# weidafeng/Efficient-SlowFast

Hardware: AMD Instinct MI355X
Metric: clips/sec (8x8 224^2 SlowFast-R50+CMDA, train step fwd+bwd+allreduce+SGD) (higher is better)
Workload: dtype f32

## Files before the change

efficient-slowfast_amd/csrc/conv_bx.hip:

```cpp
#include "bx.h"
#include <stdlib.h>

namespace {

constexpr int BXC_BM = 256;
constexpr int BXC_BK = 16;
constexpr int BXC_STAGES = 3;
constexpr int BXC_ROWB = BXC_BK * 2;
constexpr int BXC_A_STAGE = 3 * BXC_BM * BXC_ROWB;

struct BxArgs {
  sf_conv_desc d;
  const unsigned short* ap;
  const unsigned short* bp;
  float* ws;
  const float* scale;
  const float* bias;
  const float* res;
  float* out;
  int M, ntaps, cpk, nk, S, nk_per, nb_n, tiles;
  int tap_major;
  unsigned a_rows, a_bytes, b_bytes;
  unsigned a_plane, b_plane;
  unsigned wo_mul, wo_sh, ho_mul, ho_sh, to_mul, to_sh;
  const float* xf;
  unsigned xf_bytes;
  float* stats;
};

__device__ __forceinline__ unsigned mdiv(unsigned n, unsigned mul, unsigned sh) {
  return mul ? (__umulhi(n, mul) >> sh) : n;
}

typedef __attribute__((address_space(3))) void lds_void;

template <int BN, bool DIRECT, int VAR>
__global__ __launch_bounds__(512, 2) void conv_bx_kernel(const BxArgs p) {
  constexpr bool AF32 = (VAR & 32) != 0;
  constexpr int A_ST = AF32 ? BXC_BM * 64 : BXC_A_STAGE;
  constexpr int B_STAGE = 3 * BN * BXC_ROWB;
  constexpr int STAGE = A_ST + B_STAGE;
  constexpr int NT = BN / 64;
  extern __shared__ __attribute__((aligned(16))) char smem[];
  const sf_conv_desc& d = p.d;
  const int tid = threadIdx.x, lane = tid & 63;
  const int wave = __builtin_amdgcn_readfirstlane(tid >> 6);
  const int wm = wave & 3, wn = wave >> 2;
  const int bid = xcd_remap(blockIdx.x, p.tiles * p.S);
  const int split = bid / p.tiles, tile = bid - split * p.tiles;
  const int tile_m = tile / p.nb_n, tile_n = tile - tile_m * p.nb_n;
  const int m0 = tile_m * BXC_BM, n0 = tile_n * BN;
  const int ks0 = split * p.nk_per;
  const int ks1 = ks0 + p.nk_per < p.nk ? ks0 + p.nk_per : p.nk;
  const int nsteps = ks1 - ks0;

  const int lrow = lane >> 1;
  const unsigned lchunk = (unsigned)((lane & 1) ^ ((lrow >> 4) & 1)) * 16u;
  const int am = m0 + 32 * wave + lrow;
  const bool a_ok = am < p.M;
  int t0, h0, w0, nimg;
  {
    const unsigned mm = a_ok ? (unsigned)am : 0u;
    const unsigned q1 = mdiv(mm, p.wo_mul, p.wo_sh);
    const unsigned wo = mm - q1 * (unsigned)d.Wo;
    const unsigned q2 = mdiv(q1, p.ho_mul, p.ho_sh);
    const unsigned ho = q1 - q2 * (unsigned)d.Ho;
    const unsigned q3 = mdiv(q2, p.to_mul, p.to_sh);
    const unsigned to = q2 - q3 * (unsigned)d.To;
    nimg = (int)q3;
    t0 = d.transposed ? (int)to + d.pT : (int)to * d.sT - d.pT;
    h0 = d.transposed ? (int)ho + d.pH : (int)ho * d.sH - d.pH;
    w0 = d.transposed ? (int)wo + d.pW : (int)wo * d.sW - d.pW;
  }
  struct FRow { int t0, h0, w0, n; bool ok; unsigned chunk; };
  FRow fr0 = {0, 0, 0, 0, false, 0u}, fr1 = fr0;
  if constexpr (AF32) {
    auto frow = [&](int u) -> FRow {
      FRow f;
      const int r = 32 * wave + 16 * u + (lane >> 2);
      const int fm = m0 + r;
      f.ok = fm < p.M;
      f.chunk = (unsigned)((lane & 3) ^ ((r >> 2) & 3)) * 16u;
      const unsigned mm = f.ok ? (unsigned)fm : 0u;
      const unsigned q1 = mdiv(mm, p.wo_mul, p.wo_sh);
      const unsigned wo = mm - q1 * (unsigned)d.Wo;
      const unsigned q2 = mdiv(q1, p.ho_mul, p.ho_sh);
      const unsigned ho = q1 - q2 * (unsigned)d.Ho;
      const unsigned q3 = mdiv(q2, p.to_mul, p.to_sh);
      const unsigned to = q2 - q3 * (unsigned)d.To;
      f.n = (int)q3;
      f.t0 = d.transposed ? (int)to + d.pT : (int)to * d.sT - d.pT;
      f.h0 = d.transposed ? (int)ho + d.pH : (int)ho * d.sH - d.pH;
      f.w0 = d.transposed ? (int)wo + d.pW : (int)wo * d.sW - d.pW;
      return f;
    };
    fr0 = frow(0);
    fr1 = frow(1);
  }
  auto f_voff = [&](const FRow f, int kt, int kh, int kw) -> unsigned {
    const int ti = d.transposed ? f.t0 - kt * d.dT : f.t0 + kt * d.dT;
    const int hi = d.transposed ? f.h0 - kh * d.dH : f.h0 + kh * d.dH;
    const int wi = d.transposed ? f.w0 - kw * d.dW : f.w0 + kw * d.dW;
    const bool ok = f.ok && (unsigned)ti < (unsigned)d.Ti && (unsigned)hi < (unsigned)d.Hi && (unsigned)wi < (unsigned)d.Wi;
    if (!ok) return 0x80000000u;
    const unsigned r = (unsigned)(((f.n * d.Ti + ti) * d.Hi + hi) * d.Wi + wi);
    return (r * (unsigned)d.in_cs + (unsigned)d.in_coff) * 4u + f.chunk;
  };
  const unsigned row_bytes = (unsigned)d.Cin * 2u;
  auto a_voff = [&](int kt, int kh, int kw) -> unsigned {
    const int ti = d.transposed ? t0 - kt * d.dT : t0 + kt * d.dT;
    const int hi = d.transposed ? h0 - kh * d.dH : h0 + kh * d.dH;
    const int wi = d.transposed ? w0 - kw * d.dW : w0 + kw * d.dW;
    const bool ok = a_ok && (unsigned)ti < (unsigned)d.Ti && (unsigned)hi < (unsigned)d.Hi && (unsigned)wi < (unsigned)d.Wi;
    const unsigned r = ok ? (unsigned)(((nimg * d.Ti + ti) * d.Hi + hi) * d.Wi + wi) : p.a_rows;
    return r * row_bytes + lchunk;
  };
  const bool b_loader = BN == 256 || wave < BN / 32;
  const int bn = n0 + 32 * wave + lrow;
  const unsigned kbytes = (unsigned)p.nk * (unsigned)BXC_ROWB;
  const unsigned b_voff = (unsigned)((b_loader && bn < d.Cout) ? bn : d.Cout) * kbytes + lchunk;

  const __amdgpu_buffer_rsrc_t a_rs = __builtin_amdgcn_make_buffer_rsrc((void*)p.ap, 0, p.a_bytes, 0x00020000);
  const __amdgpu_buffer_rsrc_t b_rs = __builtin_amdgcn_make_buffer_rsrc((void*)p.bp, 0, p.b_bytes, 0x00020000);
  const __amdgpu_buffer_rsrc_t x_rs = __builtin_amdgcn_make_buffer_rsrc((void*)p.xf, 0, AF32 ? p.xf_bytes : 0u, 0x00020000);

  struct LS { int c, tap, kw, kh, kt; };
  LS ls;
  ls.c = __builtin_amdgcn_readfirstlane(p.tap_major ? ks0 % p.cpk : ks0 / p.ntaps);
  ls.tap = __builtin_amdgcn_readfirstlane(p.tap_major ? ks0 / p.cpk : ks0 - ls.c * p.ntaps);
  ls.kw = __builtin_amdgcn_readfirstlane(ls.tap % d.kW);
  ls.kh = __builtin_amdgcn_readfirstlane((ls.tap / d.kW) % d.kH);
  ls.kt = __builtin_amdgcn_readfirstlane(ls.tap / (d.kW * d.kH));
  const int tap_major = p.tap_major, cpk = p.cpk, kW = d.kW, kH = d.kH, kT = d.kT;
  auto next = [=](const LS o) -> LS {
    LS n;
    if (tap_major) {
      const int c1 = o.c + 1;
      const bool wc = c1 == cpk;
      n.c = wc ? 0 : c1;
      n.tap = o.tap + (wc ? 1 : 0);
      const int w1 = o.kw + (wc ? 1 : 0);
      const bool ww = w1 == kW;
      n.kw = ww ? 0 : w1;
      const int h1 = o.kh + (ww ? 1 : 0);
      const bool wh = h1 == kH;
      n.kh = wh ? 0 : h1;
      n.kt = o.kt + (wh ? 1 : 0);
      return n;
    }
    const int w1 = o.kw + 1;
    const bool ww = w1 == kW;
    n.kw = ww ? 0 : w1;
    const int h1 = o.kh + (ww ? 1 : 0);
    const bool wh = h1 == kH;
    n.kh = wh ? 0 : h1;
    const int t1 = o.kt + (wh ? 1 : 0);
    const bool wt = t1 == kT;
    n.kt = wt ? 0 : t1;
    n.tap = wt ? 0 : o.tap + 1;
    n.c = o.c + (wt ? 1 : 0);
    return n;
  };
  auto issue = [&](int stage) {
    const LS l = ls;
    unsigned cur_voff = 0, cur_aso, cur_f0 = 0, cur_f1 = 0;
    if constexpr (AF32) {
      cur_f0 = f_voff(fr0, l.kt, l.kh, l.kw);
      cur_f1 = f_voff(fr1, l.kt, l.kh, l.kw);
      cur_aso = (unsigned)l.c * 64u;
    } else {
      cur_voff = a_voff(l.kt, l.kh, l.kw);
      cur_aso = (unsigned)l.c * (unsigned)BXC_ROWB;
    }
    const unsigned cur_bso = (unsigned)(l.tap * p.cpk + l.c) * (unsigned)BXC_ROWB;
    if constexpr (AF32) {
      __builtin_amdgcn_raw_ptr_buffer_load_lds(x_rs, (lds_void*)(smem + stage * STAGE + wave * 2048), 16, cur_f0, cur_aso,
                                               0, 0);
      __builtin_amdgcn_raw_ptr_buffer_load_lds(x_rs, (lds_void*)(smem + stage * STAGE + wave * 2048 + 1024), 16, cur_f1,
                                               cur_aso, 0, 0);
    } else {
      char* const sa = smem + stage * STAGE + wave * 1024;
#pragma unroll
      for (int g = 0; g < 3; ++g)
        __builtin_amdgcn_raw_ptr_buffer_load_lds(a_rs, (lds_void*)(sa + g * (BXC_BM * BXC_ROWB)), 16, cur_voff,
                                                 cur_aso + (unsigned)g * p.a_plane, 0, 0);
    }
    if (b_loader) {
      char* const sb = smem + stage * STAGE + A_ST + wave * 1024;
#pragma unroll
      for (int g = 0; g < 3; ++g)
        __builtin_amdgcn_raw_ptr_buffer_load_lds(b_rs, (lds_void*)(sb + g * (BN * BXC_ROWB)), 16, b_voff,
                                                 cur_bso + (unsigned)g * p.b_plane, 0, 0);
    }
    ls = next(l);
  };

  const unsigned frag_lane = (unsigned)(lane & 31) * BXC_ROWB + (unsigned)(((lane >> 5) ^ ((lane >> 4) & 1)) * 16);
  const unsigned a_frag = (unsigned)(wm * 64) * BXC_ROWB + frag_lane;
  const unsigned b_frag = A_ST + (unsigned)(wn * (BN / 2)) * BXC_ROWB + frag_lane;
  unsigned f_frag[2][2] = {{0, 0}, {0, 0}};
  if constexpr (AF32) {
#pragma unroll
    for (int i = 0; i < 2; ++i) {
      const int r = wm * 64 + i * 32 + (lane & 31);
#pragma unroll
      for (int q = 0; q < 2; ++q) f_frag[i][q] = (unsigned)r * 64u + (unsigned)(((2 * (lane >> 5) + q) ^ ((r >> 2) & 3)) * 16);
    }
  }

  f32x16 acc[2][NT];
#pragma unroll
  for (int i = 0; i < 2; ++i)
#pragma unroll
    for (int j = 0; j < NT; ++j)
#pragma unroll
      for (int e = 0; e < 16; ++e) acc[i][j][e] = 0.f;

  if (nsteps > 0) issue(0);
  if (nsteps > 1) issue(1);
  for (int it = 0; it < nsteps; ++it) {
    if (it + 1 < nsteps) {
      if constexpr (AF32) {
        if (b_loader) asm volatile("s_waitcnt vmcnt(5)" ::: "memory");
        else asm volatile("s_waitcnt vmcnt(2)" ::: "memory");
      } else {
        if (b_loader) asm volatile("s_waitcnt vmcnt(6)" ::: "memory");
        else asm volatile("s_waitcnt vmcnt(3)" ::: "memory");
      }
    } else {
      asm volatile("s_waitcnt vmcnt(0)" ::: "memory");
    }
    __builtin_amdgcn_s_barrier();
    if (!(VAR & 16) && it + 2 < nsteps) issue((it + 2) % BXC_STAGES);
    const char* const st = smem + (it % BXC_STAGES) * STAGE;
    u32x4 af[2][3], bf[NT][3];
    if constexpr (AF32) {
#pragma unroll
      for (int i = 0; i < 2; ++i) {
        const f32x4 lo = *reinterpret_cast<const f32x4*>(st + f_frag[i][0]);
        const f32x4 hi = *reinterpret_cast<const f32x4*>(st + f_frag[i][1]);
        split_pair(lo[0], lo[1], af[i], 0);
        split_pair(lo[2], lo[3], af[i], 1);
        split_pair(hi[0], hi[1], af[i], 2);
        split_pair(hi[2], hi[3], af[i], 3);
      }
    }
#pragma unroll
    for (int pc = 0; pc < 3; ++pc) {
      if constexpr (!AF32) {
#pragma unroll
        for (int i = 0; i < 2; ++i)
          af[i][pc] = *reinterpret_cast<const u32x4*>(st + a_frag + pc * (BXC_BM * BXC_ROWB) + i * (32 * BXC_ROWB));
      }
#pragma unroll
      for (int j = 0; j < NT; ++j)
        bf[j][pc] = *reinterpret_cast<const u32x4*>(st + b_frag + pc * (BN * BXC_ROWB) + j * (32 * BXC_ROWB));
    }
    if (VAR & 8) {
      unsigned x = 0;
#pragma unroll
      for (int pc = 0; pc < 3; ++pc) {
#pragma unroll
        for (int i = 0; i < 2; ++i) x ^= af[i][pc][0] ^ af[i][pc][1] ^ af[i][pc][2] ^ af[i][pc][3];
#pragma unroll
        for (int j = 0; j < NT; ++j) x ^= bf[j][pc][0] ^ bf[j][pc][1] ^ bf[j][pc][2] ^ bf[j][pc][3];
      }
      acc[0][0][0] += __builtin_bit_cast(float, x & 0x007fffffu);
    } else {
#pragma unroll
      for (int i = 0; i < 2; ++i)
#pragma unroll
        for (int j = 0; j < NT; ++j) acc[i][j] = mfma_split(af[i], bf[j], acc[i][j]);
    }
  }

  const int col = lane & 31, rsub = 4 * (lane >> 5);
  if ((VAR & 4) && p.M > 0) {
    return;
  }
  if (DIRECT) {
#pragma unroll
    for (int j = 0; j < NT; ++j) {
      const int n = n0 + wn * (BN / 2) + j * 32 + col;
      const bool n_ok = n < d.Cout;
      const float sc = (p.scale && n_ok) ? p.scale[n] : 1.f;
      const float bi = (p.bias && n_ok) ? p.bias[n] : 0.f;
#pragma unroll
      for (int i = 0; i < 2; ++i) {
        float r[16];
#pragma unroll
        for (int e = 0; e < 16; ++e) {
          const int m = m0 + wm * 64 + i * 32 + (e & 3) + 8 * (e >> 2) + rsub;
          r[e] = (p.res && m < p.M && n_ok) ? p.res[(long)m * d.res_cs + d.res_coff + n] : 0.f;
        }
#pragma unroll
        for (int e = 0; e < 16; ++e) {
          const int m = m0 + wm * 64 + i * 32 + (e & 3) + 8 * (e >> 2) + rsub;
          if (m < p.M && n_ok) p.out[(long)m * d.out_cs + d.out_coff + n] = sf_act(acc[i][j][e] * sc + bi + r[e], d.act);
        }
      }
    }
    return;
  }
  float* const wsp = p.ws + (long)split * p.M * d.Cout;
#pragma unroll
  for (int i = 0; i < 2; ++i)
#pragma unroll
    for (int j = 0; j < NT; ++j) {
      const int n = n0 + wn * (BN / 2) + j * 32 + col;
#pragma unroll
      for (int e = 0; e < 16; ++e) {
        const int m = m0 + wm * 64 + i * 32 + (e & 3) + 8 * (e >> 2) + rsub;
        if (m < p.M && n < d.Cout) wsp[(long)m * d.Cout + n] = acc[i][j][e];
      }
    }
}

template <int BN, int ST>
__global__ __launch_bounds__(512, ST == 2 ? 4 : 2) void conv_pw_bx_kernel(const BxArgs p) {
  constexpr int A_STAGE = BXC_BM * 64;
  constexpr int B_STAGE = 3 * BN * BXC_ROWB;
  constexpr int STAGE = A_STAGE + B_STAGE;
  constexpr int NT = BN / 64;
  extern __shared__ __attribute__((aligned(16))) char smem[];
  const sf_conv_desc& d = p.d;
  const int tid = threadIdx.x, lane = tid & 63;
  const int wave = __builtin_amdgcn_readfirstlane(tid >> 6);
  const int wm = wave & 3, wn = wave >> 2;
  const int bid = xcd_remap(blockIdx.x, p.tiles);
  const int tile_m = bid / p.nb_n, tile_n = bid - tile_m * p.nb_n;
  const int m0 = tile_m * BXC_BM, n0 = tile_n * BN;
  const int nsteps = p.nk;

  const int lrow = lane >> 1;
  const unsigned lchunk = (unsigned)((lane & 1) ^ ((lrow >> 4) & 1)) * 16u;
  const bool b_loader = BN == 256 || wave < BN / 32;
  const int bn = n0 + 32 * wave + lrow;
  const unsigned kbytes = (unsigned)p.nk * (unsigned)BXC_ROWB;
  const unsigned b_voff = (unsigned)((b_loader && bn < d.Cout) ? bn : d.Cout) * kbytes + lchunk;
  const __amdgpu_buffer_rsrc_t b_rs = __builtin_amdgcn_make_buffer_rsrc((void*)p.bp, 0, p.b_bytes, 0x00020000);
  const __amdgpu_buffer_rsrc_t x_rs = __builtin_amdgcn_make_buffer_rsrc((void*)p.xf, 0, p.xf_bytes, 0x00020000);
  unsigned a_lvoff[2];
#pragma unroll
  for (int u = 0; u < 2; ++u) {
    const int r = 32 * wave + 16 * u + (lane >> 2);
    const int m = m0 + r;
    const unsigned chunk = (unsigned)((lane & 3) ^ ((r >> 2) & 3));
    a_lvoff[u] = m < p.M ? ((unsigned)m * (unsigned)d.in_cs + (unsigned)d.in_coff) * 4u + chunk * 16u : 0x80000000u;
  }
  auto issue = [&](int step) {
    char* const st = smem + (step % ST) * STAGE;
#pragma unroll
    for (int u = 0; u < 2; ++u)
      __builtin_amdgcn_raw_ptr_buffer_load_lds(x_rs, (lds_void*)(st + wave * 2048 + u * 1024), 16, a_lvoff[u],
                                               (unsigned)step * 64u, 0, 0);
    if (b_loader) {
      char* const sb = st + A_STAGE + wave * 1024;
#pragma unroll
      for (int g = 0; g < 3; ++g)
        __builtin_amdgcn_raw_ptr_buffer_load_lds(b_rs, (lds_void*)(sb + g * (BN * BXC_ROWB)), 16, b_voff,
                                                 (unsigned)step * (unsigned)BXC_ROWB + (unsigned)g * p.b_plane, 0, 0);
    }
  };
  unsigned a_frag[2][2];
#pragma unroll
  for (int i = 0; i < 2; ++i) {
    const int r = wm * 64 + i * 32 + (lane & 31);
#pragma unroll
    for (int q = 0; q < 2; ++q)
      a_frag[i][q] = (unsigned)r * 64u + (unsigned)(((2 * (lane >> 5) + q) ^ ((r >> 2) & 3)) * 16);
  }
  const unsigned frag_lane = (unsigned)(lane & 31) * BXC_ROWB + (unsigned)(((lane >> 5) ^ ((lane >> 4) & 1)) * 16);
  const unsigned b_frag = A_STAGE + (unsigned)(wn * (BN / 2)) * BXC_ROWB + frag_lane;

  f32x16 acc[2][NT];
#pragma unroll
  for (int i = 0; i < 2; ++i)
#pragma unroll
    for (int j = 0; j < NT; ++j)
#pragma unroll
      for (int e = 0; e < 16; ++e) acc[i][j][e] = 0.f;

  if (nsteps > 0) issue(0);
  if (ST == 3 && nsteps > 1) issue(1);
  for (int it = 0; it < nsteps; ++it) {
    if (ST == 3 && it + 1 < nsteps) {
      if (b_loader) asm volatile("s_waitcnt vmcnt(5)" ::: "memory");
      else asm volatile("s_waitcnt vmcnt(2)" ::: "memory");
    } else {
      asm volatile("s_waitcnt vmcnt(0)" ::: "memory");
    }
    __builtin_amdgcn_s_barrier();
    if (it + ST - 1 < nsteps) issue(it + ST - 1);
    const char* const st = smem + (it % ST) * STAGE;
    u32x4 af[2][3], bf[NT][3];
#pragma unroll
    for (int i = 0; i < 2; ++i) {
      const f32x4 lo = *reinterpret_cast<const f32x4*>(st + a_frag[i][0]);
      const f32x4 hi = *reinterpret_cast<const f32x4*>(st + a_frag[i][1]);
      split_pair(lo[0], lo[1], af[i], 0);
      split_pair(lo[2], lo[3], af[i], 1);
      split_pair(hi[0], hi[1], af[i], 2);
      split_pair(hi[2], hi[3], af[i], 3);
    }
#pragma unroll
    for (int pc = 0; pc < 3; ++pc)
#pragma unroll
      for (int j = 0; j < NT; ++j)
        bf[j][pc] = *reinterpret_cast<const u32x4*>(st + b_frag + pc * (BN * BXC_ROWB) + j * (32 * BXC_ROWB));
#pragma unroll
    for (int i = 0; i < 2; ++i)
#pragma unroll
      for (int j = 0; j < NT; ++j) acc[i][j] = mfma_split(af[i], bf[j], acc[i][j]);
  }

  const int col = lane & 31, rsub = 4 * (lane >> 5);
  const bool want_stats = p.stats != nullptr;
  float* const kred = reinterpret_cast<float*>(smem);
  if (want_stats) __syncthreads();
#pragma unroll
  for (int j = 0; j < NT; ++j) {
    const int cl = wn * (BN / 2) + j * 32 + col;
    const int n = n0 + cl;
    const bool n_ok = n < d.Cout;
    const float sc = (p.scale && n_ok) ? p.scale[n] : 1.f;
    const float bi = (p.bias && n_ok) ? p.bias[n] : 0.f;
#pragma unroll
    for (int i = 0; i < 2; ++i) {
      float r[16];
#pragma unroll
      for (int e = 0; e < 16; ++e) {
        const int m = m0 + wm * 64 + i * 32 + (e & 3) + 8 * (e >> 2) + rsub;
        r[e] = (p.res && m < p.M && n_ok) ? p.res[(long)m * d.res_cs + d.res_coff + n] : 0.f;
      }
#pragma unroll
      for (int e = 0; e < 16; ++e) {
        const int m = m0 + wm * 64 + i * 32 + (e & 3) + 8 * (e >> 2) + rsub;
        const float v = sf_act(acc[i][j][e] * sc + bi + r[e], d.act);
        acc[i][j][e] = v;
        if (m < p.M && n_ok) p.out[(long)m * d.out_cs + d.out_coff + n] = v;
      }
    }
    if (want_stats && wm == 0 && rsub == 0) kred[cl] = acc[0][j][0];
  }
  if (!want_stats) return;
  __syncthreads();
  float* const sred = kred + BN;
#pragma unroll
  for (int j = 0; j < NT; ++j) {
    const int cl = wn * (BN / 2) + j * 32 + col;
    const float k0 = kred[cl];
    float s1 = 0.f, s2 = 0.f;
#pragma unroll
    for (int i = 0; i < 2; ++i)
#pragma unroll
      for (int e = 0; e < 16; ++e) {
        const int m = m0 + wm * 64 + i * 32 + (e & 3) + 8 * (e >> 2) + rsub;
        if (m < p.M) {
          const float dv = acc[i][j][e] - k0;
          s1 += dv;
          s2 += dv * dv;
        }
      }
    s1 += __shfl_xor(s1, 32, 64);
    s2 += __shfl_xor(s2, 32, 64);
    if (rsub == 0) {
      sred[(wm * BN + cl) * 2] = s1;
      sred[(wm * BN + cl) * 2 + 1] = s2;
    }
  }
  __syncthreads();
  if (tid < BN) {
    const int n = n0 + tid;
    if (n < d.Cout) {
      float s1 = 0.f, s2 = 0.f;
#pragma unroll
      for (int w = 0; w < 4; ++w) {
        s1 += sred[(w * BN + tid) * 2];
        s2 += sred[(w * BN + tid) * 2 + 1];
      }
      const int left = p.M - m0;
      const float cnt = (float)(left < BXC_BM ? left : BXC_BM);
      float* const o = p.stats + ((long)tile_m * (d.Cout >> 2) + (n >> 2)) * 16 + (n & 3);
      o[0] = cnt;
      o[4] = kred[tid];
      o[8] = s1;
      o[12] = s2;
    }
  }
}

struct BxwArgs {
  sf_conv_desc d;
  const unsigned short* xp;
  const unsigned short* zp;
  float* part;
  int M, Kc, S, chunk, nb_col, tiles;
  unsigned x_rows, x_plane, x_bytes, z_plane, z_bytes;
  unsigned wo_mul, wo_sh, ho_mul, ho_sh, to_mul, to_sh, ci_mul, ci_sh;
};

__device__ __forceinline__ u32x2 lds_tr(const char* p) {
  return lds_read_tr(reinterpret_cast<const unsigned short*>(p));
}
__device__ __forceinline__ u32x2 lds_tr_raw(unsigned lds_byte_addr) {
  u32x2 r;
  asm volatile("ds_read_b64_tr_b16 %0, %1" : "=v"(r) : "v"(lds_byte_addr));
  return r;
}

template <int BCO>
__global__ __launch_bounds__(512, 2) void conv_bx_wgrad_kernel(const BxwArgs p) {
  constexpr int BCOL = 256;
  constexpr int NWC = BCO == 256 ? 2 : 4;
  constexpr int NT = BCOL / NWC / 32;
  constexpr int ROW_A = BCO * 2, ROW_B = BCOL * 2;
  constexpr int PL_A = 16 * ROW_A, PL_B = 16 * ROW_B;
  constexpr int A_STAGE = 3 * PL_A, STAGE = A_STAGE + 3 * PL_B;
  constexpr int NA = PL_A / 1024;
  constexpr int CPR_A = BCO / 8;
  extern __shared__ __attribute__((aligned(16))) char smem[];
  const sf_conv_desc& d = p.d;
  const int tid = threadIdx.x, lane = tid & 63;
  const int wave = __builtin_amdgcn_readfirstlane(tid >> 6);
  const int wr = wave / NWC, wc = wave - wr * NWC;
  const int bid = xcd_remap(blockIdx.x, p.tiles * p.S);
  const int split = bid / p.tiles, tile = bid - split * p.tiles;
  const int tile_co = tile / p.nb_col, tile_col = tile - tile_co * p.nb_col;
  const int co0 = tile_co * BCO, col0 = tile_col * BCOL;
  const int mb = split * p.chunk;
  const int me = mb + p.chunk < p.M ? mb + p.chunk : p.M;
  const int nsteps = me > mb ? (me - mb + 15) / 16 : 0;

  const int b_pos = 2 * wave + (lane >> 5);
  const int b_cs = (lane & 31) ^ ((b_pos & 3) << 2);
  const int b_col = col0 + b_cs * 8;
  const bool b_colok = b_col < p.Kc;
  const unsigned b_tap = b_colok ? mdiv((unsigned)b_col, p.ci_mul, p.ci_sh) : 0u;
  const unsigned b_ci = b_colok ? (unsigned)b_col - b_tap * (unsigned)d.Cin : 0u;
  const int b_kw = (int)(b_tap % (unsigned)d.kW), b_kh = (int)((b_tap / (unsigned)d.kW) % (unsigned)d.kH),
            b_kt = (int)(b_tap / (unsigned)(d.kW * d.kH));
  const int b_dt = b_kt * d.dT - d.pT, b_dh = b_kh * d.dH - d.pH, b_dw = b_kw * d.dW - d.pW;
  const unsigned x_rowb = (unsigned)d.Cin * 2u;
  auto b_voff = [&](int m) -> unsigned {
    unsigned r = p.x_rows;
    if (m < me && b_colok) {
      const unsigned q1 = mdiv((unsigned)m, p.wo_mul, p.wo_sh);
      const int wo = (int)((unsigned)m - q1 * (unsigned)d.Wo);
      const unsigned q2 = mdiv(q1, p.ho_mul, p.ho_sh);
      const int ho = (int)(q1 - q2 * (unsigned)d.Ho);
      const unsigned q3 = mdiv(q2, p.to_mul, p.to_sh);
      const int to = (int)(q2 - q3 * (unsigned)d.To);
      const int ti = to * d.sT + b_dt, hi = ho * d.sH + b_dh, wi = wo * d.sW + b_dw;
      if ((unsigned)ti < (unsigned)d.Ti && (unsigned)hi < (unsigned)d.Hi && (unsigned)wi < (unsigned)d.Wi)
        r = (unsigned)((((int)q3 * d.Ti + ti) * d.Hi + hi) * d.Wi + wi);
    }
    return r * x_rowb + b_ci * 2u;
  };
  const bool a_loader = wave < NA;
  const int a_pos = wave * (64 / CPR_A) + lane / CPR_A;
  const int a_cs = (lane % CPR_A) ^ ((a_pos & 3) << 2);
  const int a_co = co0 + a_cs * 8;
  const unsigned z_rowb = (unsigned)d.Cout * 2u;
  auto a_voff = [&](int m) -> unsigned {
    const unsigned r = (m < me && a_co < d.Cout) ? (unsigned)m : (unsigned)p.M;
    return r * z_rowb + (unsigned)(a_co < d.Cout ? a_co : 0) * 2u;
// ... 116 lines not shown
    } else {
      w[0] = w[1] = w[2] = (u32x4){0u, 0u, 0u, 0u};
    }
#pragma unroll
    for (int pc = 0; pc < 3; ++pc) *reinterpret_cast<u32x4*>(planes + pc * plane + r * C + c) = w[pc];
  }
}

struct BxSplitItem {
  const float* x;
  unsigned short* planes;
  long rows;
  int C, pad_;
};
__global__ __launch_bounds__(256) void bx_split_batched_kernel(const BxSplitItem* __restrict__ items,
                                                               const int* __restrict__ blk0, int n) {
  int lo = 0, hi = n;
  while (hi - lo > 1) {
    const int mid = (lo + hi) >> 1;
    if (blk0[mid] <= (int)blockIdx.x) lo = mid; else hi = mid;
  }
  const BxSplitItem it = items[lo];
  const int c8 = it.C >> 3;
  const long idx = (long)((int)blockIdx.x - blk0[lo]) * 256 + threadIdx.x;
  if (idx >= (it.rows + 1) * c8) return;
  const long plane = (it.rows + 1) * (long)it.C;
  const long r = idx / c8;
  const int c = (int)(idx - r * c8) * 8;
  u32x4 w[3];
  if (r < it.rows) {
    const f32x4 v0 = *reinterpret_cast<const f32x4*>(it.x + r * it.C + c);
    const f32x4 v1 = *reinterpret_cast<const f32x4*>(it.x + r * it.C + c + 4);
    split_pair(v0[0], v0[1], w, 0);
    split_pair(v0[2], v0[3], w, 1);
    split_pair(v1[0], v1[1], w, 2);
    split_pair(v1[2], v1[3], w, 3);
  } else {
    w[0] = w[1] = w[2] = (u32x4){0u, 0u, 0u, 0u};
  }
#pragma unroll
  for (int pc = 0; pc < 3; ++pc) *reinterpret_cast<u32x4*>(it.planes + pc * plane + r * it.C + c) = w[pc];
}

void magic(unsigned dv, unsigned* mul, unsigned* sh) {
  if (dv <= 1) { *mul = 0; *sh = 0; return; }
  unsigned l = 0;
  while ((1u << l) < dv) ++l;
  const unsigned long long num = 1ull << (31 + l);
  *mul = (unsigned)((num + dv - 1) / dv);
  *sh = l - 1;
}

int g_bx_enable = 1;
int g_bx_dbg = 0;

bool bx_enabled() {
  static const int env_on = [] {
    const char* e = getenv("SF_CONV_BX");
    return e ? atoi(e) : 1;
  }();
  return env_on && g_bx_enable;
}

struct BxPlan { int bn, S, nk, nk_per, nb_n, tiles, direct; long a_rows; };

bool bx_af32(const sf_conv_desc* d);

bool bx_plan(const sf_conv_desc* d, BxPlan* pl, bool gate = true) {
  if (!bx_enabled()) return false;
  const long M = (long)d->N * d->To * d->Ho * d->Wo;
  const int ntaps = d->kT * d->kH * d->kW;
  if ((d->Cin % 16) || d->cin_pad != d->Cin || (d->in_cs % 4) || (d->in_coff % 4)) return false;
  if (d->Cout < 128 || (d->Cout % 4) || d->out_cmul != 1) return false;
  const int nk = ntaps * (d->Cin / BXC_BK);
  if (nk < 32 || M < 2048 || M > 0x7fffffffL) return false;
  if (d->transposed && (d->sT != 1 || d->sH != 1 || d->sW != 1)) return false;
  const long a_rows = (long)d->N * d->Ti * d->Hi * d->Wi;
  if (3 * (a_rows + 1) * d->Cin * 2 > 0xfffffff0L) return false;
  if (3L * (d->Cout + 1) * nk * BXC_ROWB > 0xfffffff0L) return false;
  pl->bn = d->Cout >= 256 ? 256 : 128;
  pl->nb_n = sf_cdiv(d->Cout, pl->bn);
  pl->tiles = sf_cdiv(M, BXC_BM) * pl->nb_n;
  pl->nk = nk;
  pl->a_rows = a_rows;
  const bool scatter = d->os_T > 1 || d->os_H > 1 || d->os_W > 1;
  const double step_us = pl->bn == 256 ? 2.05 : 1.6;
  const double out_mb = (double)M * d->Cout * 4e-6;
  int best = 1;
  double best_t = 1e30;
  for (int S = 1; S <= 16 && nk / S >= 8; ++S) {
    const long wg = (long)pl->tiles * S;
    if (wg > 2048) break;
    const long rounds = sf_cdiv(wg, 256);
    double t = 6.0 + (double)rounds * sf_cdiv(nk, S) * step_us;
    if (S > 1 || scatter) t += 3.0 + out_mb * (2.0 * S + 1.0) / 4.0;
    else t += out_mb / 4.0;
    if (t < best_t - 1e-9) { best_t = t; best = S; }
  }
  static const int forced_s = [] { const char* e = getenv("SF_CONV_BX_S"); return e ? atoi(e) : 0; }();
  if (forced_s > 0 && nk / forced_s >= 1) best = forced_s;
  pl->S = best;
  pl->nk_per = sf_cdiv(nk, best);
  pl->direct = (best == 1 && !scatter) ? 1 : 0;
  if (gate && g_bx_enable < 2) {
    const double flop = 2.0 * M * (double)nk * BXC_BK * d->Cout;
    const double wave_us = flop / (nk >= 64 ? 100e6 : 90e6);
    const double split_us = bx_af32(d) ? 0.0 : 4.0 + (double)a_rows * d->Cin * 10e-6 / 3.0;
    const double pad = (double)(pl->nb_n * pl->bn) / (double)d->Cout;
    if (best_t * pad + split_us > 0.93 * wave_us) return false;
  }
  return true;
}


int g_pw_enable = 1;

struct PwPlan { int bn, nb_n, tiles, nk; };

bool pw_plan(const sf_conv_desc* d, PwPlan* pl, bool gate = true) {
  static const int env_on = [] { const char* e = getenv("SF_CONV_PW"); return e ? atoi(e) : 1; }();
  if (!bx_enabled() || !env_on || !g_pw_enable) return false;
  if (d->kT != 1 || d->kH != 1 || d->kW != 1 || d->sT != 1 || d->sH != 1 || d->sW != 1 || d->pT || d->pH || d->pW)
    return false;
  if (d->To != d->Ti || d->Ho != d->Hi || d->Wo != d->Wi) return false;
  if (d->os_T > 1 || d->os_H > 1 || d->os_W > 1 || d->out_cmul != 1) return false;
  if ((d->Cin % 16) || d->cin_pad != d->Cin || (d->in_cs % 4) || (d->in_coff % 4)) return false;
  if (d->Cin < 64 || d->Cout < 64 || (d->Cout % 4)) return false;
  const long M = (long)d->N * d->To * d->Ho * d->Wo;
  if (M < 2048 || M > 0x3fffffffL) return false;
  if (((M - 1) * d->in_cs + d->in_coff + d->Cin) * 4L >= 0x7fffffffL) return false;
  pl->nk = d->Cin / BXC_BK;
  if (3L * (d->Cout + 1) * pl->nk * BXC_ROWB > 0xfffffff0L) return false;
  static const int wide = [] { const char* e = getenv("SF_PW_WIDE"); return e ? atoi(e) : 0; }();
  static const int n64 = [] { const char* e = getenv("SF_PW_64"); return e ? atoi(e) : 1; }();
  pl->bn = (d->Cout >= 256 && wide) ? 256 : (d->Cout <= 64 ? 64 : 128);
  if (pl->bn == 64 && !n64) return false;
  pl->nb_n = sf_cdiv(d->Cout, pl->bn);
  pl->tiles = sf_cdiv(M, BXC_BM) * pl->nb_n;
  if (gate && g_pw_enable < 2 && g_bx_enable < 2) {
    const double mb = (double)M * (d->Cin + d->Cout) * 4e-6;
    if (pl->bn == 64) {
      if (d->Cin < 128) return false;
      return true;
    }
    if (d->Cout < 128) return false;
    double t_pw = 6.0 + (double)sf_cdiv(pl->tiles, 256) * pl->nk * 1.5;
    if (t_pw < mb / 4.5) t_pw = mb / 4.5;
    const double t_f32 = 6.0 + 2.0 * M * (double)d->Cin * d->Cout / 95e6 + 0.5 * mb / 4.5;
    if (t_pw > 0.85 * t_f32) return false;
  }
  return true;
}

template <int BN, int ST>
int launch_pw(const BxArgs& a, int grid, hipStream_t stream) {
  constexpr int lds = ST * (BXC_BM * 64 + 3 * BN * BXC_ROWB);
  static_assert(lds >= (BN + 4 * BN * 2) * 4, "the statistics scratch lives in the stages");
  static SfLdsAttr at;
  if (!sf_ensure_dyn_lds(at, reinterpret_cast<const void*>(conv_pw_bx_kernel<BN, ST>), lds)) return SF_ELAUNCH;
  hipLaunchKernelGGL((conv_pw_bx_kernel<BN, ST>), dim3(grid), dim3(512), lds, stream, a);
  SF_CHECK_LAUNCH();
  return SF_OK;
}

bool bx_af32(const sf_conv_desc* d) {
  static const int on = [] { const char* e = getenv("SF_CONV_BX_AF32"); return e ? atoi(e) : 1; }();
  if (!on) return false;
  const long rows = (long)d->N * d->Ti * d->Hi * d->Wi;
  return ((rows - 1) * d->in_cs + d->in_coff + d->Cin) * 4L < 0x7fffffffL;
}

long align4(long floats) { return (floats + 3) & ~3L; }
long a_plane_floats(const sf_conv_desc* d, long a_rows) { return align4((3 * (a_rows + 1) * d->Cin + 1) / 2); }
long b_plane_floats(const sf_conv_desc* d, int nk) { return align4((3L * (d->Cout + 1) * nk * BXC_BK + 1) / 2); }

template <int BN, bool DIRECT, int VAR>
int launch_bx_v(const BxArgs& a, int grid, hipStream_t stream) {
  constexpr int lds = BXC_STAGES * (((VAR & 32) ? BXC_BM * 64 : BXC_A_STAGE) + 3 * BN * BXC_ROWB);
  static SfLdsAttr at;
  if (!sf_ensure_dyn_lds(at, reinterpret_cast<const void*>(conv_bx_kernel<BN, DIRECT, VAR>), lds)) return SF_ELAUNCH;
  hipLaunchKernelGGL((conv_bx_kernel<BN, DIRECT, VAR>), dim3(grid), dim3(512), lds, stream, a);
  SF_CHECK_LAUNCH();
  return SF_OK;
}

template <int BN, bool DIRECT>
int launch_bx(const BxArgs& a, int grid, hipStream_t stream) {
  static const int var = [] { const char* e = getenv("SF_CONV_BX_VAR"); return e ? atoi(e) : 0; }();
  if (a.xf) return launch_bx_v<BN, DIRECT, 32>(a, grid, stream);
  switch (var) {
    case 4: return launch_bx_v<BN, DIRECT, 4>(a, grid, stream);
    case 12: return launch_bx_v<BN, DIRECT, 12>(a, grid, stream);
    case 20: return launch_bx_v<BN, DIRECT, 20>(a, grid, stream);
    case 28: return launch_bx_v<BN, DIRECT, 28>(a, grid, stream);
    default: return launch_bx_v<BN, DIRECT, 0>(a, grid, stream);
  }
}

}

int sf_conv_bx_tune(int value) { g_bx_enable = value; return SF_OK; }
int sf_conv_bx_dbg(int value) { g_bx_dbg = value; return SF_OK; }

int sf_conv_bx_takes(const sf_conv_desc* d) {
  BxPlan pl;
  return bx_plan(d, &pl) ? 1 : 0;
}

extern "C" long sf_bx_planes_elems(long rows, int C) { return 3 * (rows + 1) * (long)C; }

int sf_bx_split_rows(const float* x, int cs, int coff, long rows, int C, unsigned short* planes, hipStream_t s) {
  if ((C & 7) || (cs & 3) || (coff & 3) || !sf_aligned16(x) || !sf_aligned16(planes)) return SF_EALIGN;
  const long total = (rows + 1) * (C >> 3);
  long blocks = (total + 255) / 256;
  if (blocks > 256 * 16) blocks = 256 * 16;
  hipLaunchKernelGGL(bx_split_rows_kernel, dim3((unsigned)blocks), dim3(256), 0, s, x, cs, coff, rows, C, planes);
  SF_CHECK_LAUNCH();
  return SF_OK;
}

extern "C" int sf_bx_split(const float* x, int cs, int coff, long rows, int C, unsigned short* planes, void* stream) {
  if (!x || !planes || rows <= 0 || C <= 0) return SF_EINVAL;
  return sf_bx_split_rows(x, cs, coff, rows, C, planes, (hipStream_t)stream);
}

extern "C" int sf_bx_split_batched(const void* items, const int* blk0, int n, int nblocks, void* stream) {
  if (!items || !blk0 || n <= 0 || nblocks <= 0) return SF_EINVAL;
  hipLaunchKernelGGL(bx_split_batched_kernel, dim3(nblocks), dim3(256), 0, (hipStream_t)stream,
                     reinterpret_cast<const BxSplitItem*>(items), blk0, n);
  SF_CHECK_LAUNCH();
  return SF_OK;
}

int sf_conv_pw_tune(int value) { g_pw_enable = value; return SF_OK; }

int sf_conv_pw_takes(const sf_conv_desc* d) {
  PwPlan pl;
  return pw_plan(d, &pl) ? 1 : 0;
}

extern "C" long sf_conv_pw_ws_floats(const sf_conv_desc* d, int have_w_planes) {
  PwPlan pl;
  if (!d || !pw_plan(d, &pl)) return 0;
  return 4 + (have_w_planes ? 0 : b_plane_floats(d, pl.nk));
}

extern "C" long sf_conv_pw_stats_floats(const sf_conv_desc* d) {
  PwPlan pl;
  if (!d || d->transposed || d->act != SF_ACT_NONE || !pw_plan(d, &pl)) return 0;
  const long M = (long)d->N * d->To * d->Ho * d->Wo;
  return (long)sf_cdiv(M, BXC_BM) * 4 * d->Cout;
}

int sf_conv_pw_try(const sf_conv_desc* d, const float* in, const float* w_packed, const unsigned short* w_planes,
                   const float* scale, const float* bias, const float* res, float* out, float* ws, float* stats,
                   int* parts, hipStream_t stream) {
  PwPlan pl;
  if (parts) *parts = 0;
  if (!ws || !pw_plan(d, &pl)) return 1;
  if (!sf_aligned16(in) || !sf_aligned16(w_packed) || !sf_aligned16(ws)) return 1;
  if (w_planes && !sf_aligned16(w_planes)) return SF_EALIGN;
  if (stats && (scale || res || d->act != SF_ACT_NONE || !parts || !sf_aligned16(stats))) return 1;
  const long M = (long)d->N * d->To * d->Ho * d->Wo;
  if (!w_planes) {
    unsigned short* const bp = reinterpret_cast<unsigned short*>(ws + 4);
    const int rc = sf_bx_split_rows(w_packed, pl.nk * BXC_BK, 0, d->Cout, pl.nk * BXC_BK, bp, stream);
    if (rc != SF_OK) return rc;
    w_planes = bp;
  }
  BxArgs a = {};
  a.d = *d;
  a.bp = w_planes;
  a.scale = scale; a.bias = bias; a.res = res; a.out = out;
  a.M = (int)M;
  a.ntaps = 1; a.cpk = pl.nk; a.nk = pl.nk; a.S = 1; a.nk_per = pl.nk; a.nb_n = pl.nb_n; a.tiles = pl.tiles;
  a.b_plane = (unsigned)((long)(d->Cout + 1) * pl.nk * BXC_ROWB);
  a.b_bytes = 3u * a.b_plane;
  a.xf = in;
  a.xf_bytes = (unsigned)(((M - 1) * d->in_cs + d->in_coff + d->Cin) * 4L);
  a.stats = stats;
  if (stats) *parts = (int)sf_cdiv(M, BXC_BM);
  if (pl.bn == 256) return launch_pw<256, 3>(a, pl.tiles, stream);
  if (pl.bn == 64) return launch_pw<64, 2>(a, pl.tiles, stream);
  return launch_pw<128, 2>(a, pl.tiles, stream);
}

extern "C" int sf_conv_fwd_pw(const sf_conv_desc* d, const float* in, const float* w_packed,
                              const unsigned short* w_planes, const float* scale, const float* bias, const float* res,
                              float* out, float* ws, float* stats, int* parts, void* stream) {
  if (!d || !in || !w_packed || !out || !ws) return SF_EINVAL;
  const int rc = sf_conv_pw_try(d, in, w_packed, w_planes, scale, bias, res, out, ws, stats, parts, (hipStream_t)stream);
  return rc == 1 ? SF_ENOTTAKEN : rc;
}

extern "C" long sf_conv_bx_ws_floats(const sf_conv_desc* d, int have_in_planes, int have_w_planes) {
  BxPlan pl;
  if (!d || !bx_plan(d, &pl)) return 0;
  const long M = (long)d->N * d->To * d->Ho * d->Wo;
  return 4 + ((have_in_planes || bx_af32(d)) ? 0 : a_plane_floats(d, pl.a_rows)) +
         (have_w_planes ? 0 : b_plane_floats(d, pl.nk)) + (pl.direct ? 0 : (long)pl.S * M * d->Cout);
}

int sf_conv_splitk_finish(const sf_conv_desc* d, const float* ws, int S, const float* scale, const float* bias,
                          const float* res, float* out, hipStream_t s);

int sf_conv_bx_try(const sf_conv_desc* d, const float* in, const unsigned short* in_planes, const float* w_packed,
                   const unsigned short* w_planes, const float* scale, const float* bias, const float* res, float* out,
                   float* ws, hipStream_t stream) {
  BxPlan pl;
  if (!ws || !bx_plan(d, &pl)) return 1;
  if (!sf_aligned16(in) || !sf_aligned16(w_packed) || !sf_aligned16(ws)) return 1;
  if ((in_planes && !sf_aligned16(in_planes)) || (w_planes && !sf_aligned16(w_planes))) return SF_EALIGN;
  const long M = (long)d->N * d->To * d->Ho * d->Wo;
  float* cur = ws;
  int rc = SF_OK;
  const bool af32 = bx_af32(d);
  if (!in_planes && !af32) {
    unsigned short* const ap = reinterpret_cast<unsigned short*>(cur);
    cur += a_plane_floats(d, pl.a_rows);
    if (!(g_bx_dbg & 1)) rc = sf_bx_split_rows(in, d->in_cs, d->in_coff, pl.a_rows, d->Cin, ap, stream);
    if (rc != SF_OK) return rc;
    in_planes = ap;
  }
  if (!w_planes) {
    unsigned short* const bp = reinterpret_cast<unsigned short*>(cur);
    cur += b_plane_floats(d, pl.nk);
    if (!(g_bx_dbg & 1)) rc = sf_bx_split_rows(w_packed, pl.nk * BXC_BK, 0, d->Cout, pl.nk * BXC_BK, bp, stream);
    if (rc != SF_OK) return rc;
    w_planes = bp;
  }
  BxArgs a = {};
  a.d = *d;
  a.ap = in_planes; a.bp = w_planes; a.ws = cur;
  if (af32) {
    a.xf = in;
    a.xf_bytes = (unsigned)(((pl.a_rows - 1) * d->in_cs + d->in_coff + d->Cin) * 4L);
  }
  a.scale = scale; a.bias = bias; a.res = res; a.out = out;
  a.M = (int)M;
  a.ntaps = d->kT * d->kH * d->kW;
  a.cpk = d->Cin / BXC_BK;
  a.nk = pl.nk; a.S = pl.S; a.nk_per = pl.nk_per; a.nb_n = pl.nb_n; a.tiles = pl.tiles;
  a.tap_major = (d->sT > 1 || d->sH > 1 || d->sW > 1) ? 1 : 0;
  a.a_rows = (unsigned)pl.a_rows;
  a.a_plane = (unsigned)((pl.a_rows + 1) * d->Cin * 2);
  a.a_bytes = 3u * a.a_plane;
  a.b_plane = (unsigned)((long)(d->Cout + 1) * pl.nk * BXC_ROWB);
  a.b_bytes = 3u * a.b_plane;
  magic((unsigned)d->Wo, &a.wo_mul, &a.wo_sh);
  magic((unsigned)d->Ho, &a.ho_mul, &a.ho_sh);
  magic((unsigned)d->To, &a.to_mul, &a.to_sh);
  const int grid = pl.tiles * pl.S;
  if (!(g_bx_dbg & 4)) {
    if (pl.bn == 256) rc = pl.direct ? launch_bx<256, true>(a, grid, stream) : launch_bx<256, false>(a, grid, stream);
    else rc = pl.direct ? launch_bx<128, true>(a, grid, stream) : launch_bx<128, false>(a, grid, stream);
    if (rc != SF_OK) return rc;
  }
  if (pl.direct || (g_bx_dbg & 2)) return SF_OK;
  return sf_conv_splitk_finish(d, cur, pl.S, scale, bias, res, out, stream);
}

extern "C" int sf_conv_fwd_bx(const sf_conv_desc* d, const float* in, const unsigned short* in_planes,
                              const float* w_packed, const unsigned short* w_planes, const float* scale,
                              const float* bias, const float* res, float* out, float* ws, void* stream) {
  if (!d || !in || !w_packed || !out || !ws) return SF_EINVAL;
  const int rc = sf_conv_bx_try(d, in, in_planes, w_packed, w_planes, scale, bias, res, out, ws, (hipStream_t)stream);
  return rc == 1 ? SF_ENOTTAKEN : rc;
}

namespace {

struct BxwPlan { int bco, S, nb_col, tiles; long chunk, x_rows; };

int g_bxw_enable = 1;

bool bxw_plan(const sf_conv_desc* d, BxwPlan* pl) {
  static const int env_on = [] { const char* e = getenv("SF_WGRAD_BX"); return e ? atoi(e) : 1; }();
  if (!env_on || !g_bxw_enable) return false;
  const long M = (long)d->N * d->To * d->Ho * d->Wo;
  const int ntaps = d->kT * d->kH * d->kW;
  if ((d->Cin % 8) || d->cin_pad != d->Cin || (d->in_cs % 4) || (d->in_coff % 4)) return false;
  if (d->Cout < 128 || (d->Cout % 8)) return false;
  const long Kc = (long)ntaps * d->Cin;
  if (Kc < 512 || M < 2048 || M > 0x7ffffff0L) return false;
  const long x_rows = (long)d->N * d->Ti * d->Hi * d->Wi;
  if (3 * (x_rows + 1) * d->Cin * 2 > 0xfffffff0L || 3 * (M + 1) * d->Cout * 2 > 0xfffffff0L) return false;
  pl->bco = d->Cout >= 256 ? 256 : 128;
  pl->nb_col = sf_cdiv(Kc, 256);
  pl->tiles = sf_cdiv(d->Cout, pl->bco) * pl->nb_col;
  pl->x_rows = x_rows;
  const double step_us = pl->bco == 256 ? 2.0 : 1.1;
  const double out_mb = (double)d->Cout * Kc * 4e-6;
  int best = 1;
  double best_t = 1e30;
  const int maxS = (int)(M / 256 > 512 ? 512 : M / 256);
  for (int S = 1; S <= maxS; ++S) {
    const long wg = (long)pl->tiles * S;
    if (wg > 1536) break;
    const long rounds = sf_cdiv(wg, 256);
    const long steps = sf_cdiv(sf_cdiv(M, S), 16);
    const double t = 6.0 + (double)rounds * steps * step_us + out_mb * (2.0 * S + 1.0) / 4.0;
    if (t < best_t - 1e-9) { best_t = t; best = S; }
  }
  static const int forced_s = [] { const char* e = getenv("SF_WGRAD_BX_S"); return e ? atoi(e) : 0; }();
  if (forced_s > 0) best = forced_s;
  pl->S = best;
  pl->chunk = (sf_cdiv(M, best) + 15) / 16 * 16;
  if (g_bxw_enable < 2) {
    const double flop = 2.0 * M * (double)Kc * d->Cout;
    const double wave_us = flop / 95e6;
    const double split_us = 8.0 + ((double)x_rows * d->Cin + (double)M * d->Cout) * 10e-6 / 3.0;
    if (best_t + split_us > 0.93 * wave_us) return false;
  }
  return true;
}

long x_plane_floats(const sf_conv_desc* d, long x_rows) { return align4((3 * (x_rows + 1) * d->Cin + 1) / 2); }
long z_plane_floats(const sf_conv_desc* d, long M) { return align4((3 * (M + 1) * d->Cout + 1) / 2); }

template <int BCO>
int launch_bxw(const BxwArgs& a, int grid, hipStream_t stream) {
  constexpr int lds = BXC_STAGES * (3 * 16 * BCO * 2 + 3 * 16 * 256 * 2);
  static SfLdsAttr at;
  if (!sf_ensure_dyn_lds(at, reinterpret_cast<const void*>(conv_bx_wgrad_kernel<BCO>), lds)) return SF_ELAUNCH;
  hipLaunchKernelGGL((conv_bx_wgrad_kernel<BCO>), dim3(grid), dim3(512), lds, stream, a);
  SF_CHECK_LAUNCH();
  return SF_OK;
}

}

int sf_conv_bxw_tune(int value) { g_bxw_enable = value; return SF_OK; }

extern "C" int sf_conv_wgrad_bx_splits(const sf_conv_desc* d) {
  BxwPlan pl;
  return (d && bxw_plan(d, &pl)) ? pl.S : 0;
}
// ... 54 lines not shown
```

Before: 149.2.

## Generalize conv K-loop into configurable LDS ring with multi-step consume chunks

Rewrites the main K loops of the bx and pointwise conv kernels as a generic ring buffer. RING slots are prefetched ahead and CS steps are consumed per barrier, with vmcnt waits derived from how far ahead loads are outstanding. Ring depth and chunk size are template parameters, chosen through new environment variables. By default the f32-input bx kernel with BN below 256 now uses a 2-slot ring with doubled occupancy in its launch bounds, instead of 3 stages. This trades deeper prefetch for more resident blocks to hide latency, at the cost of a full memory wait on every step.

Result: no change. 148.9, median of 6 (-0.2%).

```diff
diff --git a/efficient-slowfast_amd/csrc/conv_bx.hip b/efficient-slowfast_amd/csrc/conv_bx.hip
--- a/efficient-slowfast_amd/csrc/conv_bx.hip
+++ b/efficient-slowfast_amd/csrc/conv_bx.hip
@@ -6,6 +6,7 @@
 constexpr int BXC_BM = 256;
 constexpr int BXC_BK = 16;
 constexpr int BXC_STAGES = 3;
+constexpr int BXC_LDS = 160 * 1024;
 constexpr int BXC_ROWB = BXC_BK * 2;
 constexpr int BXC_A_STAGE = 3 * BXC_BM * BXC_ROWB;
 
@@ -34,13 +35,31 @@
 
 typedef __attribute__((address_space(3))) void lds_void;
 
-template <int BN, bool DIRECT, int VAR>
-__global__ __launch_bounds__(512, 2) void conv_bx_kernel(const BxArgs p) {
+template <int N>
+__device__ __forceinline__ void vm_wait() {
+  asm volatile("s_waitcnt vmcnt(%0)" ::"n"(N) : "memory");
+}
+template <int MAXA, int L>
+__device__ __forceinline__ void ring_wait(int ahead) {
+  if constexpr (MAXA >= 2) {
+    if (ahead >= 2) { vm_wait<2 * L>(); return; }
+  }
+  if constexpr (MAXA >= 1) {
+    if (ahead >= 1) { vm_wait<L>(); return; }
+  }
+  vm_wait<0>();
+}
+
+
+template <int BN, bool DIRECT, int VAR, int RING, int CS>
+__global__ __launch_bounds__(512, 2 * RING * (((VAR & 32) ? BXC_BM * 64 : BXC_A_STAGE) + 3 * BN * BXC_ROWB) <= BXC_LDS ? 4 : 2)
+void conv_bx_kernel(const BxArgs p) {
   constexpr bool AF32 = (VAR & 32) != 0;
   constexpr int A_ST = AF32 ? BXC_BM * 64 : BXC_A_STAGE;
   constexpr int B_STAGE = 3 * BN * BXC_ROWB;
   constexpr int STAGE = A_ST + B_STAGE;
   constexpr int NT = BN / 64;
+  static_assert(RING * STAGE <= BXC_LDS && RING >= 2 * CS, "ring of conv_bx_kernel");
   extern __shared__ __attribute__((aligned(16))) char smem[];
   const sf_conv_desc& d = p.d;
   const int tid = threadIdx.x, lane = tid & 63;
@@ -216,23 +235,8 @@
 #pragma unroll
       for (int e = 0; e < 16; ++e) acc[i][j][e] = 0.f;
 
-  if (nsteps > 0) issue(0);
-  if (nsteps > 1) issue(1);
-  for (int it = 0; it < nsteps; ++it) {
-    if (it + 1 < nsteps) {
-      if constexpr (AF32) {
-        if (b_loader) asm volatile("s_waitcnt vmcnt(5)" ::: "memory");
-        else asm volatile("s_waitcnt vmcnt(2)" ::: "memory");
-      } else {
-        if (b_loader) asm volatile("s_waitcnt vmcnt(6)" ::: "memory");
-        else asm volatile("s_waitcnt vmcnt(3)" ::: "memory");
-      }
-    } else {
-      asm volatile("s_waitcnt vmcnt(0)" ::: "memory");
-    }
-    __builtin_amdgcn_s_barrier();
-    if (!(VAR & 16) && it + 2 < nsteps) issue((it + 2) % BXC_STAGES);
-    const char* const st = smem + (it % BXC_STAGES) * STAGE;
+  auto consume = [&](int slot) {
+    const char* const st = smem + slot * STAGE;
     u32x4 af[2][3], bf[NT][3];
     if constexpr (AF32) {
 #pragma unroll
@@ -272,6 +276,34 @@
 #pragma unroll
         for (int j = 0; j < NT; ++j) acc[i][j] = mfma_split(af[i], bf[j], acc[i][j]);
     }
+  };
+
+  constexpr int LA = AF32 ? 2 : 3;
+  int issued = 0, islot = 0, cslot = 0;
+  auto issue_next = [&]() {
+    issue(islot);
+    ++issued;
+    islot = islot + 1 == RING ? 0 : islot + 1;
+  };
+#pragma unroll
+  for (int s = 0; s < RING - CS; ++s)
+    if (s < nsteps) issue_next();
+  for (int k0 = 0; k0 < nsteps; k0 += CS) {
+    const int kend = k0 + CS < nsteps ? k0 + CS : nsteps;
+    if (b_loader) ring_wait<RING - 2 * CS, LA + 3>(issued - kend);
+    else ring_wait<RING - 2 * CS, LA>(issued - kend);
+    __builtin_amdgcn_s_barrier();
+    if (!(VAR & 16)) {
+      const int lim = k0 + RING < nsteps ? k0 + RING : nsteps;
+#pragma unroll
+      for (int u = 0; u < CS; ++u)
+        if (issued < lim) issue_next();
+    }
+#pragma unroll
+    for (int u = 0; u < CS; ++u) {
+      if (u == 0 || k0 + u < nsteps) consume(cslot);
+      cslot = cslot + 1 == RING ? 0 : cslot + 1;
+    }
   }
 
   const int col = lane & 31, rsub = 4 * (lane >> 5);
@@ -316,12 +348,17 @@
     }
 }
 
-template <int BN, int ST>
-__global__ __launch_bounds__(512, ST == 2 ? 4 : 2) void conv_pw_bx_kernel(const BxArgs p) {
+template <int BN, int RING, int CS>
+constexpr int pw_lds() { return RING * (BXC_BM * 64 + 3 * BN * BXC_ROWB); }
+
+template <int BN, int RING, int CS>
+__global__ __launch_bounds__(512, 2 * RING * (BXC_BM * 64 + 3 * BN * BXC_ROWB) <= BXC_LDS ? 4 : 2)
+void conv_pw_bx_kernel(const BxArgs p) {
   constexpr int A_STAGE = BXC_BM * 64;
   constexpr int B_STAGE = 3 * BN * BXC_ROWB;
   constexpr int STAGE = A_STAGE + B_STAGE;
   constexpr int NT = BN / 64;
+  static_assert(RING * STAGE <= BXC_LDS && RING >= 2 * CS, "ring of conv_pw_bx_kernel");
   extern __shared__ __attribute__((aligned(16))) char smem[];
   const sf_conv_desc& d = p.d;
   const int tid = threadIdx.x, lane = tid & 63;
@@ -348,8 +385,8 @@
     const unsigned chunk = (unsigned)((lane & 3) ^ ((r >> 2) & 3));
     a_lvoff[u] = m < p.M ? ((unsigned)m * (unsigned)d.in_cs + (unsigned)d.in_coff) * 4u + chunk * 16u : 0x80000000u;
   }
-  auto issue = [&](int step) {
-    char* const st = smem + (step % ST) * STAGE;
+  auto issue = [&](int step, int slot) {
+    char* const st = smem + slot * STAGE;
 #pragma unroll
     for (int u = 0; u < 2; ++u)
       __builtin_amdgcn_raw_ptr_buffer_load_lds(x_rs, (lds_void*)(st + wave * 2048 + u * 1024), 16, a_lvoff[u],
@@ -381,18 +418,8 @@
 #pragma unroll
       for (int e = 0; e < 16; ++e) acc[i][j][e] = 0.f;
 
-  if (nsteps > 0) issue(0);
-  if (ST == 3 && nsteps > 1) issue(1);
-  for (int it = 0; it < nsteps; ++it) {
-    if (ST == 3 && it + 1 < nsteps) {
-      if (b_loader) asm volatile("s_waitcnt vmcnt(5)" ::: "memory");
-      else asm volatile("s_waitcnt vmcnt(2)" ::: "memory");
-    } else {
-      asm volatile("s_waitcnt vmcnt(0)" ::: "memory");
-    }
-    __builtin_amdgcn_s_barrier();
-    if (it + ST - 1 < nsteps) issue(it + ST - 1);
-    const char* const st = smem + (it % ST) * STAGE;
+  auto consume = [&](int slot) {
+    const char* const st = smem + slot * STAGE;
     u32x4 af[2][3], bf[NT][3];
 #pragma unroll
     for (int i = 0; i < 2; ++i) {
@@ -412,6 +439,30 @@
     for (int i = 0; i < 2; ++i)
 #pragma unroll
       for (int j = 0; j < NT; ++j) acc[i][j] = mfma_split(af[i], bf[j], acc[i][j]);
+  };
+  int issued = 0, islot = 0, cslot = 0;
+  auto issue_next = [&]() {
+    issue(issued, islot);
+    ++issued;
+    islot = islot + 1 == RING ? 0 : islot + 1;
+  };
+#pragma unroll
+  for (int s = 0; s < RING - CS; ++s)
+    if (s < nsteps) issue_next();
+  for (int k0 = 0; k0 < nsteps; k0 += CS) {
+    const int kend = k0 + CS < nsteps ? k0 + CS : nsteps;
+    if (b_loader) ring_wait<RING - 2 * CS, 5>(issued - kend);
+    else ring_wait<RING - 2 * CS, 2>(issued - kend);
+    __builtin_amdgcn_s_barrier();
+    const int lim = k0 + RING < nsteps ? k0 + RING : nsteps;
+#pragma unroll
+    for (int u = 0; u < CS; ++u)
+      if (issued < lim) issue_next();
+#pragma unroll
+    for (int u = 0; u < CS; ++u) {
+      if (u == 0 || k0 + u < nsteps) consume(cslot);
+      cslot = cslot + 1 == RING ? 0 : cslot + 1;
+    }
   }
 
   const int col = lane & 31, rsub = 4 * (lane >> 5);
@@ -834,15 +885,36 @@
   return true;
 }
 
-template <int BN, int ST>
-int launch_pw(const BxArgs& a, int grid, hipStream_t stream) {
-  constexpr int lds = ST * (BXC_BM * 64 + 3 * BN * BXC_ROWB);
+template <int BN, int RING, int CS>
+int launch_pw_v(const BxArgs& a, int grid, hipStream_t stream) {
+  constexpr int lds = pw_lds<BN, RING, CS>();
   static_assert(lds >= (BN + 4 * BN * 2) * 4, "the statistics scratch lives in the stages");
   static SfLdsAttr at;
-  if (!sf_ensure_dyn_lds(at, reinterpret_cast<const void*>(conv_pw_bx_kernel<BN, ST>), lds)) return SF_ELAUNCH;
-  hipLaunchKernelGGL((conv_pw_bx_kernel<BN, ST>), dim3(grid), dim3(512), lds, stream, a);
+  if (!sf_ensure_dyn_lds(at, reinterpret_cast<const void*>(conv_pw_bx_kernel<BN, RING, CS>), lds)) return SF_ELAUNCH;
+  hipLaunchKernelGGL((conv_pw_bx_kernel<BN, RING, CS>), dim3(grid), dim3(512), lds, stream, a);
   SF_CHECK_LAUNCH();
   return SF_OK;
+}
+
+int ring_env(const char* name) {
+  const char* e = getenv(name);
+  return e ? atoi(e) : 0;
+}
+
+template <int BN>
+int launch_pw(const BxArgs& a, int grid, hipStream_t stream) {
+  static const int ring = ring_env("SF_CONV_PW_RING");
+  if constexpr (BN == 256) {
+    if (ring == 42) return launch_pw_v<256, 4, 2>(a, grid, stream);
+    return launch_pw_v<256, 3, 1>(a, grid, stream);
+  } else {
+    switch (ring) {
+      case 31: return launch_pw_v<BN, 3, 1>(a, grid, stream);
+      case 42: return launch_pw_v<BN, 4, 2>(a, grid, stream);
+      case 52: return launch_pw_v<BN, 5, 2>(a, grid, stream);
+      default: return launch_pw_v<BN, 2, 1>(a, grid, stream);
+    }
+  }
 }
 
 bool bx_af32(const sf_conv_desc* d) {
@@ -856,12 +928,13 @@
 long a_plane_floats(const sf_conv_desc* d, long a_rows) { return align4((3 * (a_rows + 1) * d->Cin + 1) / 2); }
 long b_plane_floats(const sf_conv_desc* d, int nk) { return align4((3L * (d->Cout + 1) * nk * BXC_BK + 1) / 2); }
 
-template <int BN, bool DIRECT, int VAR>
+template <int BN, bool DIRECT, int VAR, int RING = 3, int CS = 1>
 int launch_bx_v(const BxArgs& a, int grid, hipStream_t stream) {
-  constexpr int lds = BXC_STAGES * (((VAR & 32) ? BXC_BM * 64 : BXC_A_STAGE) + 3 * BN * BXC_ROWB);
+  constexpr int lds = RING * (((VAR & 32) ? BXC_BM * 64 : BXC_A_STAGE) + 3 * BN * BXC_ROWB);
   static SfLdsAttr at;
-  if (!sf_ensure_dyn_lds(at, reinterpret_cast<const void*>(conv_bx_kernel<BN, DIRECT, VAR>), lds)) return SF_ELAUNCH;
-  hipLaunchKernelGGL((conv_bx_kernel<BN, DIRECT, VAR>), dim3(grid), dim3(512), lds, stream, a);
+  if (!sf_ensure_dyn_lds(at, reinterpret_cast<const void*>(conv_bx_kernel<BN, DIRECT, VAR, RING, CS>), lds))
+    return SF_ELAUNCH;
+  hipLaunchKernelGGL((conv_bx_kernel<BN, DIRECT, VAR, RING, CS>), dim3(grid), dim3(512), lds, stream, a);
   SF_CHECK_LAUNCH();
   return SF_OK;
 }
@@ -869,7 +942,21 @@
 template <int BN, bool DIRECT>
 int launch_bx(const BxArgs& a, int grid, hipStream_t stream) {
   static const int var = [] { const char* e = getenv("SF_CONV_BX_VAR"); return e ? atoi(e) : 0; }();
-  if (a.xf) return launch_bx_v<BN, DIRECT, 32>(a, grid, stream);
+  if (a.xf) {
+    static const int ring = ring_env("SF_CONV_BX_RING");
+    if constexpr (BN == 256) {
+      if (ring == 41) return launch_bx_v<BN, DIRECT, 32, 4, 1>(a, grid, stream);
+      if (ring == 42) return launch_bx_v<BN, DIRECT, 32, 4, 2>(a, grid, stream);
+      return launch_bx_v<BN, DIRECT, 32, 3, 1>(a, grid, stream);
+    } else {
+      switch (ring) {
+        case 31: return launch_bx_v<BN, DIRECT, 32, 3, 1>(a, grid, stream);
+        case 42: return launch_bx_v<BN, DIRECT, 32, 4, 2>(a, grid, stream);
+        case 52: return launch_bx_v<BN, DIRECT, 32, 5, 2>(a, grid, stream);
+        default: return launch_bx_v<BN, DIRECT, 32, 2, 1>(a, grid, stream);
+      }
+    }
+  }
   switch (var) {
     case 4: return launch_bx_v<BN, DIRECT, 4>(a, grid, stream);
     case 12: return launch_bx_v<BN, DIRECT, 12>(a, grid, stream);
@@ -962,9 +1049,9 @@
   a.xf_bytes = (unsigned)(((M - 1) * d->in_cs + d->in_coff + d->Cin) * 4L);
   a.stats = stats;
   if (stats) *parts = (int)sf_cdiv(M, BXC_BM);
-  if (pl.bn == 256) return launch_pw<256, 3>(a, pl.tiles, stream);
-  if (pl.bn == 64) return launch_pw<64, 2>(a, pl.tiles, stream);
-  return launch_pw<128, 2>(a, pl.tiles, stream);
+  if (pl.bn == 256) return launch_pw<256>(a, pl.tiles, stream);
+  if (pl.bn == 64) return launch_pw<64>(a, pl.tiles, stream);
+  return launch_pw<128>(a, pl.tiles, stream);
 }
 
 extern "C" int sf_conv_fwd_pw(const sf_conv_desc* d, const float* in, const float* w_packed,
```
